# ZhengyiLuo/PULSE

Hardware: NVIDIA H100
Metric: env-steps/sec at 16384 humanoid envs, 1/2/4/8 H100; obs-kernel HBM GB/s (higher is better)
Workload: dtype bf16 GEMM operands, fp32 accumulate / master weights / observations

## Files before the change

pulse_b200/csrc/gemm_kernel.inc:

```
#if PULSE_GEMM_GROUPED
#define PULSE_GEMM_FIRST(member) grp.p[0].member
#define PULSE_GEMM_W wl
#define PULSE_GEMM_SELECT(w)                                                                                         \
  int pi = 0;                                                                                                        \
  while (pi + 1 < grp.count && (w) >= grp.p[pi].item_end) ++pi;                                                      \
  const GemmProblem& P = grp.p[pi];                                                                                  \
  const int wl = (w) - (pi == 0 ? 0 : grp.p[pi - 1].item_end);                                                       \
  const CUtensorMap& map_a = P.map_a;                                                                                \
  const CUtensorMap& map_b = P.map_b;                                                                                \
  const CUtensorMap& map_c = P.map_c;                                                                                \
  const int use_tma_red = P.use_tma_red;                                                                             \
  const pulse_gemm_epilogue_t& ep = P.ep;                                                                            \
  const int M = P.M, N = P.N, K = P.K, kb_per_split = P.kb_per_split;                                                \
  const int tiles_n = (N + BN - 1) / BN, tiles_m = (M + BM - 1) / BM;                                                \
  const int tiles = tiles_m * tiles_n;                                                                               \
  const int num_kb_total = (K + BK - 1) / BK;                                                                        \
  (void)map_a; (void)map_b; (void)map_c; (void)use_tma_red; (void)ep; (void)M; (void)N; (void)tiles_n; (void)kb_per_split; (void)num_kb_total;
#else
#define PULSE_GEMM_FIRST(member) member
#define PULSE_GEMM_W w
#define PULSE_GEMM_SELECT(w)
#endif

#if PULSE_GEMM_GROUPED
// ... 19 lines not shown
  const int work_stride = static_cast<int>(gridDim.x);
#if PULSE_GEMM_GROUPED
  const int total = grp.total_items;
#else
  const int tiles_n = (N + BN - 1) / BN, tiles_m = (M + BM - 1) / BM;
  const int tiles = tiles_m * tiles_n;
  const int total = tiles * splits;
  const int num_kb_total = (K + BK - 1) / BK;
#endif
  if (threadIdx.x == 0) PULSE_TRACE(0);

  if (threadIdx.x == 0) {
#pragma unroll
    for (int s = 0; s < kStages; ++s) {
      g_mbar_init(&sm.full[s], 1);
      g_mbar_init(&sm.empty[s], kConsumerWarps);
    }
    asm volatile("fence.mbarrier_init.release.cluster;\n" ::: "memory");
    asm volatile("prefetch.tensormap [%0];\n" ::"l"(&PULSE_GEMM_FIRST(map_a)) : "memory");
    asm volatile("prefetch.tensormap [%0];\n" ::"l"(&PULSE_GEMM_FIRST(map_b)) : "memory");
  }
  __syncthreads();
  if (threadIdx.x == 0) PULSE_TRACE(1);
  asm volatile("griddepcontrol.launch_dependents;\n" ::: "memory");

  if (warp < 4) {
    if (warp == 0 && lane == 0) {
      asm volatile("griddepcontrol.wait;\n" ::: "memory");
      PULSE_TRACE(2);
      int it = 0;
      for (int w = work0; w < total; w += work_stride) {
        PULSE_GEMM_SELECT(w)
        const int split = PULSE_GEMM_W / tiles, t = PULSE_GEMM_W - split * tiles;
        const int m0 = (t / tiles_n) * BM, n0 = (t % tiles_n) * BN;
        const int kb0 = split * kb_per_split;
        const int num_kb = min(kb_per_split, num_kb_total - kb0);
        for (int kb = 0; kb < num_kb; ++kb, ++it) {
          const int s = it % kStages;
          g_mbar_wait(&sm.empty[s], ((it / kStages) & 1) ^ 1);
          g_mbar_expect_tx(&sm.full[s], kStageBytesA + kStageBytesB);
          const int kk = (kb0 + kb) * BK;
// ... 1 lines not shown
            tma_load_2d(sm.a[s], &map_a, m0, kk, &sm.full[s]);
            tma_load_2d(sm.a[s] + 8192, &map_a, m0 + 64, kk, &sm.full[s]);
          } else {
            tma_load_2d(sm.a[s], &map_a, kk, m0, &sm.full[s]);
          }
          if (B_MN) {
            tma_load_2d(sm.b[s], &map_b, n0, kk, &sm.full[s]);
            tma_load_2d(sm.b[s] + 8192, &map_b, n0 + 64, kk, &sm.full[s]);
          } else {
            tma_load_2d(sm.b[s], &map_b, kk, n0, &sm.full[s]);
          }
        }
      }
    }
  } else {
    const int wg = (warp >> 2) - 1;
    const int ew = warp - 4;
    const int quarter = wg * 2 + (warp & 1);
    const int chalf = (warp >> 1) & 1;
    float* red_stage = sm.red[ew];
    float* acc_s = sm.acc[wg];
    asm volatile("griddepcontrol.wait;\n" ::: "memory");
    int it = 0, lw = 0;
    for (int w = work0; w < total; w += work_stride, ++lw) {
      PULSE_GEMM_SELECT(w)
      const int split = PULSE_GEMM_W / tiles, t = PULSE_GEMM_W - split * tiles;
      const int m0 = (t / tiles_n) * BM, n0 = (t % tiles_n) * BN;
      const int kb0 = split * kb_per_split;
      const int num_kb = min(kb_per_split, num_kb_total - kb0);
      const int row = m0 + quarter * 32 + lane;
      const bool row_ok = row < M;
      const bool gate_fast = (MODE == kModeGeneric || MODE == kModeDgrad) && ep.gate != nullptr && ep.gate_mask == nullptr && ep.gate_mode == PULSE_ACT_RELU && (ep.ldg & 7) == 0 && n0 + chalf * kCols + kCols <= N;
      unsigned gmask[kChunks] = {};
      const bool gate_bits = kDgrad && ep.gate_mask != nullptr;
      if (gate_bits && row_ok) {
#pragma unroll
        for (int cc = 0; cc < kChunks; ++cc) {
          const int col = n0 + (chalf * kChunks + cc) * 32;
          if (col < N) gmask[cc] = __ldg(ep.gate_mask + static_cast<long long>(col >> 5) * ep.ld_gmask + row);
        }
      }
      if (gate_fast && row_ok) {
        const uint4* g = reinterpret_cast<const uint4*>(reinterpret_cast<const __nv_bfloat16*>(ep.gate) + static_cast<long long>(row) * ep.ldg +
                                                        n0 + chalf * kCols);
        uint4 u[kChunks * 4];
#pragma unroll
        for (int i = 0; i < kChunks * 4; ++i) u[i] = __ldg(g + i);
#pragma unroll
        for (int i = 0; i < kChunks * 4; ++i) {
          const unsigned wds[4] = {u[i].x, u[i].y, u[i].z, u[i].w};
#pragma unroll
          for (int q = 0; q < 4; ++q) {
            const unsigned pos = (((wds[q] & 0x7fff7fffu) + 0x7fff7fffu) & ~wds[q]) & 0x80008000u;
            gmask[i >> 2] |= (pos >> 15) << ((i & 3) * 4 + q);
          }
        }
      }
      const bool gate_vec = kGateVec && ep.gate != nullptr && !gate_fast && !gate_bits && (ep.ldg & 7) == 0;
      uint4 gq[4] = {};
      auto gate_fetch = [&](int cc) {
        const int c0 = n0 + cc * 32;
        if (gate_vec && row_ok && c0 + 32 <= N) {
          const uint4* g = reinterpret_cast<const uint4*>(reinterpret_cast<const __nv_bfloat16*>(ep.gate) + static_cast<long long>(row) * ep.ldg + c0);
#pragma unroll
          for (int q = 0; q < 4; ++q) gq[q] = __ldg(g + q);
        }
      };
      gate_fetch(chalf * kChunks);
      float bias_l[kChunks] = {};
      const bool fwd_fast = MODE == kModeFwd && ep.out != nullptr && (ep.ldo & 7) == 0 && ep.out_f32 == nullptr && ep.out_t == nullptr &&
                            (ep.preact == nullptr || (ep.ldp & 7) == 0) && n0 + chalf * kCols + kCols <= N;
      float* bias_s = sm.bias[ew];
      if (fwd_fast && ep.bias != nullptr) {
        __syncwarp();
#pragma unroll
        for (int cc = 0; cc < kChunks; ++cc) bias_s[cc * 32 + lane] = __ldg(ep.bias + n0 + (chalf * kChunks + cc) * 32 + lane);
        __syncwarp();
      } else if (kFwd && ep.bias != nullptr) {
#pragma unroll
        for (int cc = 0; cc < kChunks; ++cc) {
          const int col = n0 + (chalf * kChunks + cc) * 32 + lane;
          if (col < N) bias_l[cc] = __ldg(ep.bias + col);
        }
      }

      float d[64];
#pragma unroll
      for (int i = 0; i < 64; ++i) d[i] = 0.0f;
      acc_fence(d);
      int prev_s = -1;
      for (int kb = 0; kb < num_kb; ++kb, ++it) {
        const int s = it % kStages;
        g_mbar_wait(&sm.full[s], (it / kStages) & 1);
        if (it == 0 && ew == 0 && lane == 0) PULSE_TRACE(3);
        wgmma_fence();
        const unsigned a_addr = s_u32(sm.a[s]) + static_cast<unsigned>(wg) * 8192u, b_addr = s_u32(sm.b[s]);
#pragma unroll
        for (int k = 0; k < BK / MMA_K; ++k) {
          const unsigned long long da = A_MN ? gmma_desc(a_addr + k * 2048, 8192) : gmma_desc(a_addr + k * 32, 16);
          const unsigned long long db = B_MN ? gmma_desc(b_addr + k * 2048, 8192) : gmma_desc(b_addr + k * 32, 16);
          wgmma_m64n128<A_MN ? 1 : 0, B_MN ? 1 : 0>(d, da, db, (kb | k) != 0 ? 1u : 0u);
        }
        wgmma_commit();
        wgmma_wait<1>();
        if (prev_s >= 0 && lane == 0) g_mbar_arrive(&sm.empty[prev_s]);
        prev_s = s;
      }
      wgmma_wait<0>();
      acc_fence(d);
      if (lane == 0) g_mbar_arrive(&sm.empty[prev_s]);
      if (ew == 0 && lane == 0 && lw < 3) PULSE_TRACE(4 + lw);

      wg_sync(wg);
      {
        const int r0 = (warp & 3) * 16 + (lane >> 2);
#pragma unroll
        for (int j = 0; j < BN / 8; ++j) {
          const int col = 8 * j + 2 * (lane & 3);
#pragma unroll
          for (int h = 0; h < 2; ++h) {
            const int r = r0 + 8 * h;
            const int rb = r & 31;
            float* blk = acc_s + ((r >> 5) * 4 + (col >> 5)) * 1024;
            const int unit = ((col & 31) >> 2) ^ (rb & 7);
            *reinterpret_cast<float2*>(blk + rb * 32 + unit * 4 + (col & 3)) = make_float2(d[4 * j + 2 * h], d[4 * j + 2 * h + 1]);
          }
        }
      }
      if (MODE == kModeWgrad && use_tma_red) asm volatile("fence.proxy.async.shared::cta;\n" ::: "memory");
      wg_sync(wg);
      if (ew == 0 && lane == 0 && lw < 3) PULSE_TRACE(16 + 2 * lw);

      float* outf = ep.out_f32 != nullptr ? ep.out_f32 + static_cast<long long>(ep.accumulate ? 0 : split) * ep.split_stride : nullptr;
      float sq = 0.0f;
#pragma unroll 1
      for (int c = chalf * kChunks; c < chalf * kChunks + kChunks; ++c) {
        const int col0 = n0 + c * 32;
        const bool full = col0 + 32 <= N;
        float* blk = acc_s + ((quarter & 1) * 4 + c) * 1024;
        if (MODE == kModeWgrad && use_tma_red) {
          if (lane == 0) {
            asm volatile("cp.reduce.async.bulk.tensor.2d.global.shared::cta.add.tile.bulk_group [%0, {%2, %3}], [%1];\n" ::"l"(&map_c),
                         "r"(s_u32(blk)), "r"(col0), "r"(m0 + quarter * 32)
                         : "memory");
            asm volatile("cp.async.bulk.commit_group;\n" ::: "memory");
          }
          continue;
        }
        float v[32];
        {
          const float4* b4 = reinterpret_cast<const float4*>(blk) + lane * 8;
#pragma unroll
          for (int u = 0; u < 8; ++u) {
            const float4 x = b4[u ^ (lane & 7)];
            v[4 * u] = x.x; v[4 * u + 1] = x.y; v[4 * u + 2] = x.z; v[4 * u + 3] = x.w;
          }
        }
        if (MODE != kModeWgrad && ep.alpha != 1.0f) {
#pragma unroll
          for (int i = 0; i < 32; ++i) v[i] *= ep.alpha;
        }
        if (fwd_fast) {
          if (ep.bias != nullptr) {
            const float4* b4 = reinterpret_cast<const float4*>(bias_s + (c % kChunks) * 32);
#pragma unroll
            for (int i = 0; i < 32; i += 4) {
              const float4 b = b4[i >> 2];
              v[i] += b.x; v[i + 1] += b.y; v[i + 2] += b.z; v[i + 3] += b.w;
            }
          }
          if (ep.relu_mask != nullptr) {
            unsigned word = 0u;
#pragma unroll
            for (int i = 0; i < 32; ++i) word |= (v[i] > 0.0f ? 1u : 0u) << i;
            if (row_ok) ep.relu_mask[static_cast<long long>(col0 >> 5) * ep.ld_rmask + row] = word;
          }
          uint4* st = reinterpret_cast<uint4*>(red_stage);
          const int sw = (lane >> 1) & 3;
#pragma unroll
          for (int q = 0; q < 4; ++q) {
            const int i = 8 * q;
            __nv_bfloat162 h0 = __floats2bfloat162_rn(v[i], v[i + 1]), h1 = __floats2bfloat162_rn(v[i + 2], v[i + 3]);
            __nv_bfloat162 h2 = __floats2bfloat162_rn(v[i + 4], v[i + 5]), h3 = __floats2bfloat162_rn(v[i + 6], v[i + 7]);
            uint4 u;
            u.x = *reinterpret_cast<unsigned*>(&h0);
            u.y = *reinterpret_cast<unsigned*>(&h1);
            u.z = *reinterpret_cast<unsigned*>(&h2);
            u.w = *reinterpret_cast<unsigned*>(&h3);
            st[lane * 4 + (q ^ sw)] = u;
          }
          __syncwarp();
          const long long coff = col0 + (lane & 3) * 8;
          const __nv_bfloat162 zero2 = __float2bfloat162_rn(0.0f);
#pragma unroll
          for (int it2 = 0; it2 < 4; ++it2) {
            const int rr = it2 * 8 + (lane >> 2);
            uint4 u = st[rr * 4 + ((lane & 3) ^ ((rr >> 1) & 3))];
            __nv_bfloat162* h = reinterpret_cast<__nv_bfloat162*>(&u);
            const long long grow = m0 + quarter * 32 + rr;
            if (grow < M) {
              if (ep.preact != nullptr) *reinterpret_cast<uint4*>(reinterpret_cast<__nv_bfloat16*>(ep.preact) + grow * ep.ldp + coff) = u;
              if (ep.act == PULSE_ACT_RELU) {
#pragma unroll
                for (int q = 0; q < 4; ++q) h[q] = __hmax2(h[q], zero2);
              } else if (ep.act == PULSE_ACT_SILU) {
#pragma unroll
                for (int q = 0; q < 4; ++q) h[q] = silu_bf16x2(h[q]);
              }
              *reinterpret_cast<uint4*>(reinterpret_cast<__nv_bfloat16*>(ep.out) + grow * ep.ldo + coff) = u;
            }
          }
          __syncwarp();
          continue;
        }
        if (kFwd && ep.bias != nullptr) {
          float bl = bias_l[0];
#pragma unroll
          for (int cc = 1; cc < kChunks; ++cc) bl = (c % kChunks) == cc ? bias_l[cc] : bl;
#pragma unroll
          for (int i = 0; i < 32; ++i) v[i] += __shfl_sync(0xffffffffu, bl, i);
        }
        if (kFwd && ep.preact != nullptr) {
          if (full && (ep.ldp & 7) == 0) {
            store_block_bf16(reinterpret_cast<uint4*>(red_stage), v,
                             reinterpret_cast<__nv_bfloat16*>(ep.preact) + static_cast<long long>(m0 + quarter * 32) * ep.ldp + col0, ep.ldp,
                             M - (m0 + quarter * 32), lane);
          } else if (row_ok) {
            __nv_bfloat16* p = reinterpret_cast<__nv_bfloat16*>(ep.preact) + static_cast<long long>(row) * ep.ldp + col0;
#pragma unroll
            for (int i = 0; i < 32; ++i)
              if (col0 + i < N) p[i] = __float2bfloat16(v[i]);
          }
        }
        if (kFwd && ep.relu_mask != nullptr && row_ok) {
          unsigned word = 0u;
#pragma unroll
          for (int i = 0; i < 32; ++i) word |= ((col0 + i < N && v[i] > 0.0f) ? 1u : 0u) << i;
          if (col0 < N) ep.relu_mask[static_cast<long long>(col0 >> 5) * ep.ld_rmask + row] = word;
        }
        if (kFwd && ep.act != PULSE_ACT_NONE) {
#pragma unroll
          for (int i = 0; i < 32; ++i) v[i] = act_apply(v[i], ep.act);
        }
        if (gate_bits) {
          unsigned mk = gmask[0];
#pragma unroll
          for (int cc = 1; cc < kChunks; ++cc) mk = (c % kChunks) == cc ? gmask[cc] : mk;
#pragma unroll
          for (int i = 0; i < 32; ++i) v[i] = ((mk >> i) & 1u) ? v[i] : 0.0f;
        } else if (gate_fast) {
          unsigned mk = gmask[0];
#pragma unroll
          for (int cc = 1; cc < kChunks; ++cc) mk = (c % kChunks) == cc ? gmask[cc] : mk;
#pragma unroll
          for (int i = 0; i < 32; ++i) v[i] = ((mk >> ((i >> 1) + 16 * (i & 1))) & 1u) ? v[i] : 0.0f;
        } else if (kDgrad && ep.gate != nullptr && row_ok) {
          const __nv_bfloat16* g = reinterpret_cast<const __nv_bfloat16*>(ep.gate) + static_cast<long long>(row) * ep.ldg + col0;
          if (full && (gate_vec || (ep.ldg & 7) == 0)) {
#pragma unroll
            for (int i = 0; i < 32; i += 8) {
              const uint4 u = gate_vec ? gq[i >> 3] : __ldg(reinterpret_cast<const uint4*>(g + i));
              const __nv_bfloat162* h = reinterpret_cast<const __nv_bfloat162*>(&u);
#pragma unroll
              for (int q = 0; q < 4; ++q) {
                const float2 f = __bfloat1622float2(h[q]);
                v[i + 2 * q] *= act_grad(f.x, ep.gate_mode);
                v[i + 2 * q + 1] *= act_grad(f.y, ep.gate_mode);
              }
            }
          } else {
#pragma unroll
            for (int i = 0; i < 32; ++i)
              if (col0 + i < N) v[i] *= act_grad(__bfloat162float(g[i]), ep.gate_mode);
          }
        }
        if (gate_vec && c != chalf * kChunks + kChunks - 1) gate_fetch(c + 1);
        if (kDgrad && ep.sumsq != nullptr && row_ok) {
#pragma unroll
          for (int i = 0; i < 32; ++i)
            if (full || col0 + i < N) sq = fmaf(v[i], v[i], sq);
        }
        if (kDgrad && ep.colsum != nullptr) {
          float wv[32];
#pragma unroll
          for (int i = 0; i < 32; ++i) wv[i] = row_ok ? v[i] : 0.0f;
#pragma unroll
          for (int half = 16; half >= 1; half >>= 1) {
            const bool upper = (lane & half) != 0;
#pragma unroll
            for (int i = 0; i < half; ++i) {
              const float mine = upper ? wv[i + half] : wv[i];
              const float send = upper ? wv[i] : wv[i + half];
              wv[i] = mine + __shfl_xor_sync(0xffffffffu, send, half);
            }
          }
          if (col0 + lane < N) atomicAdd(ep.colsum + col0 + lane, wv[0]);
        }
        if (kAccum && outf != nullptr && ep.accumulate) {
#pragma unroll
          for (int hr = 0; hr < 2; ++hr) {
            if ((lane >> 4) == hr) {
#pragma unroll
              for (int i = 0; i < 32; ++i) red_stage[(lane & 15) * 33 + i] = v[i];
            }
            __syncwarp();
            const int rbase = m0 + quarter * 32 + hr * 16;
            const int rows_here = min(16, M - rbase);
            if (col0 + lane < N) {
              float* p = outf + static_cast<long long>(rbase) * ep.ldf + col0 + lane;
              for (int rr = 0; rr < rows_here; ++rr) atomicAdd(p + static_cast<long long>(rr) * ep.ldf, red_stage[rr * 33 + lane]);
            }
            __syncwarp();
          }
        } else if (outf != nullptr && row_ok) {
          float* p = outf + static_cast<long long>(row) * ep.ldf + col0;
          if (full && (ep.ldf & 3) == 0 && (reinterpret_cast<uintptr_t>(outf) & 15u) == 0) {
#pragma unroll
            for (int i = 0; i < 32; i += 4) *reinterpret_cast<float4*>(p + i) = make_float4(v[i], v[i + 1], v[i + 2], v[i + 3]);
          } else {
#pragma unroll
            for (int i = 0; i < 32; ++i)
              if (col0 + i < N) p[i] = v[i];
          }
        }
        if (kBf16Out && ep.out != nullptr) {
          if (full && (ep.ldo & 7) == 0) {
            store_block_bf16(reinterpret_cast<uint4*>(red_stage), v,
                             reinterpret_cast<__nv_bfloat16*>(ep.out) + static_cast<long long>(m0 + quarter * 32) * ep.ldo + col0, ep.ldo,
                             M - (m0 + quarter * 32), lane);
          } else if (row_ok) {
            __nv_bfloat16* p = reinterpret_cast<__nv_bfloat16*>(ep.out) + static_cast<long long>(row) * ep.ldo + col0;
#pragma unroll
            for (int i = 0; i < 32; ++i)
              if (col0 + i < N) p[i] = __float2bfloat16(v[i]);
          }
        }
        if (kFwd && ep.out_t != nullptr && row_ok) {
#pragma unroll
          for (int i = 0; i < 32; ++i)
            if (col0 + i < N)
              reinterpret_cast<__nv_bfloat16*>(ep.out_t)[static_cast<long long>(col0 + i) * ep.ldot + row] = __float2bfloat16(v[i]);
        }
      }
      if (MODE == kModeWgrad && use_tma_red) {
        if (lane == 0) asm volatile("cp.async.bulk.wait_group.read 0;\n" ::: "memory");
        __syncwarp();
      }
      if (kDgrad && ep.sumsq != nullptr) {
#pragma unroll
        for (int o = 16; o > 0; o >>= 1) sq += __shfl_xor_sync(0xffffffffu, sq, o);
        if (lane == 0) atomicAdd(ep.sumsq, static_cast<double>(sq));
      }
      if (ew == 0 && lane == 0 && lw < 3) PULSE_TRACE(17 + 2 * lw);
    }
  }
  if (MODE == kModeWgrad && warp >= 4 && lane == 0) asm volatile("cp.async.bulk.wait_group 0;\n" ::: "memory");
  if (threadIdx.x == 0) PULSE_TRACE(10);
}


#undef PULSE_GEMM_FIRST
#undef PULSE_GEMM_W
#undef PULSE_GEMM_SELECT
```

pulse_b200/csrc/gemm_wgmma.cu:

```cuda
#include <cuda.h>
#include <stdlib.h>
#include <string.h>
#include <cuda_bf16.h>

#include "pulse_common.cuh"

namespace pulse {
namespace {

#ifndef PULSE_GEMM_VARIANT
#define PULSE_GEMM_VARIANT 0
#endif
constexpr int BM = 128, BN = 128, BK = 64, MMA_K = 16;
constexpr int kConsumerWarps = 8;
constexpr int kThreads = 128 + 32 * kConsumerWarps;
constexpr int kCols = 64;
constexpr int kChunks = kCols / 32;
constexpr int kStages = 4;
constexpr unsigned kStageBytesA = BM * BK * 2;
constexpr unsigned kStageBytesB = BN * BK * 2;

struct __align__(1024) GemmSmem {
  unsigned char a[kStages][kStageBytesA];
  unsigned char b[kStages][kStageBytesB];
  float acc[2][64 * BN];
  float red[kConsumerWarps][16 * 33];
  float bias[kConsumerWarps][kCols];
  unsigned long long full[kStages];
  unsigned long long empty[kStages];
};

__device__ __forceinline__ unsigned s_u32(const void* p) { return static_cast<unsigned>(__cvta_generic_to_shared(p)); }
__device__ __forceinline__ void g_mbar_init(unsigned long long* bar, unsigned count) {
  asm volatile("mbarrier.init.shared::cta.b64 [%0], %1;\n" ::"r"(s_u32(bar)), "r"(count));
}
__device__ __forceinline__ void g_mbar_expect_tx(unsigned long long* bar, unsigned bytes) {
  asm volatile("mbarrier.arrive.expect_tx.shared::cta.b64 _, [%0], %1;\n" ::"r"(s_u32(bar)), "r"(bytes) : "memory");
}
__device__ __forceinline__ void g_mbar_arrive(unsigned long long* bar) {
  asm volatile("mbarrier.arrive.shared::cta.b64 _, [%0];\n" ::"r"(s_u32(bar)) : "memory");
}
__device__ __forceinline__ bool g_mbar_try(unsigned long long* bar, unsigned parity) {
// ... 86 lines not shown
    u.z = *reinterpret_cast<unsigned*>(&h2);
    u.w = *reinterpret_cast<unsigned*>(&h3);
    st[lane * 4 + (q ^ sw)] = u;
  }
  __syncwarp();
  __nv_bfloat16* obase = base + (lane & 3) * 8;
#pragma unroll
  for (int it = 0; it < 4; ++it) {
    const int rr = it * 8 + (lane >> 2);
    const uint4 val = st[rr * 4 + ((lane & 3) ^ ((rr >> 1) & 3))];
    if (rr < rows_valid) *reinterpret_cast<uint4*>(obase + static_cast<long long>(rr) * ld) = val;
  }
  __syncwarp();
}

#if PULSE_GEMM_VARIANT == 3
__device__ long long g_gemm_trace[32];
#define PULSE_TRACE(slot)                                          \
  do {                                                             \
    if (blockIdx.x == 0) g_gemm_trace[slot] = clock64();           \
  } while (0)
#else
#define PULSE_TRACE(slot) \
  do {                    \
  } while (0)
#endif

__device__ __forceinline__ __nv_bfloat162 silu_bf16x2(__nv_bfloat162 z) {
  float2 f = __bfloat1622float2(z);
  f.x = __fdividef(f.x, 1.0f + __expf(-f.x));
// ... 52 lines not shown
bool make_map_c(CUtensorMap* map, const float* base, long long rows, long long cols, long long ld) {
  EncodeTiledFn fn = get_encode_fn();
  if (fn == nullptr) return false;
  cuuint64_t dims[2] = {static_cast<cuuint64_t>(cols), static_cast<cuuint64_t>(rows)};
  cuuint64_t strides[1] = {static_cast<cuuint64_t>(ld) * 4};
  cuuint32_t box[2] = {32, 32};
  cuuint32_t estr[2] = {1, 1};
  return fn(map, CU_TENSOR_MAP_DATA_TYPE_FLOAT32, 2, const_cast<float*>(base), dims, strides, box, estr, CU_TENSOR_MAP_INTERLEAVE_NONE,
            CU_TENSOR_MAP_SWIZZLE_128B, CU_TENSOR_MAP_L2_PROMOTION_NONE, CU_TENSOR_MAP_FLOAT_OOB_FILL_NONE) == CUDA_SUCCESS;
}
bool tma_reduce_ok(const pulse_gemm_epilogue_t& ep) {
  return ep.out_f32 != nullptr && ep.accumulate && (ep.ldf % 4) == 0 && (reinterpret_cast<uintptr_t>(ep.out_f32) % 16) == 0;
}

constexpr size_t kSmemBytes = sizeof(GemmSmem) + 1024;

int gemm_num_sms(bool honour_limit) {
  static int num_sms = 0, limited = 0;
  if (num_sms == 0) {
    int dev = 0;
    if (cudaGetDevice(&dev) != cudaSuccess || cudaDeviceGetAttribute(&num_sms, cudaDevAttrMultiProcessorCount, dev) != cudaSuccess) return 0;
    limited = num_sms;
    const char* e = getenv("PULSE_GEMM_SMS");
    if (e != nullptr && atoi(e) >= 1 && atoi(e) < num_sms) limited = atoi(e);
  }
  return honour_limit ? limited : num_sms;
}

template <bool A_MN, bool B_MN, int MODE>
int launch_gemm(const CUtensorMap& map_a, const CUtensorMap& map_b, const pulse_gemm_epilogue_t& ep, int m, int n, int k, int splits,
// ... 212 lines not shown
```

Before: 1.456 million.

## Ping-pong consumer warpgroups with 128-row tiles and register-direct epilogue

Each consumer warpgroup now handles whole alternating tiles and computes both 64-row halves (two accumulators) instead of splitting one tile across warpgroups. Named barriers order the two groups so one runs its MMAs while the other runs its epilogue. setmaxnreg moves registers from the producer to the consumers to fit the doubled accumulators. A new register-only epilogue for forward and dgrad writes bf16 outputs through quad shuffles without staging in shared memory, which also frees the red/bias shared buffers. The risks are register pressure or spills, and the change to the empty-barrier count and the barrier handshake must be correct.

```diff
diff --git a/pulse_b200/csrc/gemm_kernel.inc b/pulse_b200/csrc/gemm_kernel.inc
--- a/pulse_b200/csrc/gemm_kernel.inc
+++ b/pulse_b200/csrc/gemm_kernel.inc
@@ -57,7 +57,7 @@
 #pragma unroll
     for (int s = 0; s < kStages; ++s) {
       g_mbar_init(&sm.full[s], 1);
-      g_mbar_init(&sm.empty[s], kConsumerWarps);
+      g_mbar_init(&sm.empty[s], 4);
     }
     asm volatile("fence.mbarrier_init.release.cluster;\n" ::: "memory");
     asm volatile("prefetch.tensormap [%0];\n" ::"l"(&PULSE_GEMM_FIRST(map_a)) : "memory");
@@ -68,6 +68,7 @@
   asm volatile("griddepcontrol.launch_dependents;\n" ::: "memory");
 
   if (warp < 4) {
+    asm volatile("setmaxnreg.dec.sync.aligned.u32 %0;\n" ::"n"(kProducerRegs));
     if (warp == 0 && lane == 0) {
       asm volatile("griddepcontrol.wait;\n" ::: "memory");
       PULSE_TRACE(2);
@@ -99,11 +100,10 @@
       }
     }
   } else {
+    asm volatile("setmaxnreg.inc.sync.aligned.u32 %0;\n" ::"n"(kConsumerRegs));
     const int wg = (warp >> 2) - 1;
     const int ew = warp - 4;
-    const int quarter = wg * 2 + (warp & 1);
     const int chalf = (warp >> 1) & 1;
-    float* red_stage = sm.red[ew];
     float* acc_s = sm.acc[wg];
     asm volatile("griddepcontrol.wait;\n" ::: "memory");
     int it = 0, lw = 0;
@@ -113,330 +113,368 @@
       const int m0 = (t / tiles_n) * BM, n0 = (t % tiles_n) * BN;
       const int kb0 = split * kb_per_split;
       const int num_kb = min(kb_per_split, num_kb_total - kb0);
-      const int row = m0 + quarter * 32 + lane;
-      const bool row_ok = row < M;
-      const bool gate_fast = (MODE == kModeGeneric || MODE == kModeDgrad) && ep.gate != nullptr && ep.gate_mask == nullptr && ep.gate_mode == PULSE_ACT_RELU && (ep.ldg & 7) == 0 && n0 + chalf * kCols + kCols <= N;
-      unsigned gmask[kChunks] = {};
-      const bool gate_bits = kDgrad && ep.gate_mask != nullptr;
-      if (gate_bits && row_ok) {
-#pragma unroll
-        for (int cc = 0; cc < kChunks; ++cc) {
-          const int col = n0 + (chalf * kChunks + cc) * 32;
-          if (col < N) gmask[cc] = __ldg(ep.gate_mask + static_cast<long long>(col >> 5) * ep.ld_gmask + row);
-        }
-      }
-      if (gate_fast && row_ok) {
-        const uint4* g = reinterpret_cast<const uint4*>(reinterpret_cast<const __nv_bfloat16*>(ep.gate) + static_cast<long long>(row) * ep.ldg +
-                                                        n0 + chalf * kCols);
-        uint4 u[kChunks * 4];
-#pragma unroll
-        for (int i = 0; i < kChunks * 4; ++i) u[i] = __ldg(g + i);
-#pragma unroll
-        for (int i = 0; i < kChunks * 4; ++i) {
-          const unsigned wds[4] = {u[i].x, u[i].y, u[i].z, u[i].w};
-#pragma unroll
-          for (int q = 0; q < 4; ++q) {
-            const unsigned pos = (((wds[q] & 0x7fff7fffu) + 0x7fff7fffu) & ~wds[q]) & 0x80008000u;
-            gmask[i >> 2] |= (pos >> 15) << ((i & 3) * 4 + q);
-          }
-        }
-      }
-      const bool gate_vec = kGateVec && ep.gate != nullptr && !gate_fast && !gate_bits && (ep.ldg & 7) == 0;
-      uint4 gq[4] = {};
-      auto gate_fetch = [&](int cc) {
-        const int c0 = n0 + cc * 32;
-        if (gate_vec && row_ok && c0 + 32 <= N) {
-          const uint4* g = reinterpret_cast<const uint4*>(reinterpret_cast<const __nv_bfloat16*>(ep.gate) + static_cast<long long>(row) * ep.ldg + c0);
-#pragma unroll
-          for (int q = 0; q < 4; ++q) gq[q] = __ldg(g + q);
+      if ((lw & 1) != wg) {
+        it += num_kb;
+        continue;
+      }
+
+      const bool reg_fwd = MODE == kModeFwd && ep.out != nullptr && (ep.ldo & 7) == 0 && ep.out_f32 == nullptr && ep.out_t == nullptr &&
+                           (ep.preact == nullptr || (ep.ldp & 7) == 0) && n0 + BN <= N;
+      const bool reg_dgrad = MODE == kModeDgrad && ep.out != nullptr && (ep.ldo & 7) == 0 && ep.out_f32 == nullptr && ep.gate_mask != nullptr &&
+                             ep.gate == nullptr && ep.colsum == nullptr && ep.sumsq == nullptr && n0 + BN <= N;
+      const int row_r = m0 + 16 * (warp & 3) + (lane >> 2);
+      float2 bias2[BN / 8] = {};
+      unsigned gm[2][2][BN / 32] = {};
+      auto load_gate_words = [&](int half) {
+#pragma unroll
+        for (int hr = 0; hr < 2; ++hr) {
+          const int r = row_r + 64 * half + 8 * hr;
+#pragma unroll
+          for (int cc = 0; cc < BN / 32; ++cc)
+            if (r < M) gm[half][hr][cc] = __ldg(ep.gate_mask + static_cast<long long>((n0 >> 5) + cc) * ep.ld_gmask + r);
         }
       };
-      gate_fetch(chalf * kChunks);
-      float bias_l[kChunks] = {};
-      const bool fwd_fast = MODE == kModeFwd && ep.out != nullptr && (ep.ldo & 7) == 0 && ep.out_f32 == nullptr && ep.out_t == nullptr &&
-                            (ep.preact == nullptr || (ep.ldp & 7) == 0) && n0 + chalf * kCols + kCols <= N;
-      float* bias_s = sm.bias[ew];
-      if (fwd_fast && ep.bias != nullptr) {
-        __syncwarp();
-#pragma unroll
-        for (int cc = 0; cc < kChunks; ++cc) bias_s[cc * 32 + lane] = __ldg(ep.bias + n0 + (chalf * kChunks + cc) * 32 + lane);
-        __syncwarp();
-      } else if (kFwd && ep.bias != nullptr) {
-#pragma unroll
-        for (int cc = 0; cc < kChunks; ++cc) {
-          const int col = n0 + (chalf * kChunks + cc) * 32 + lane;
-          if (col < N) bias_l[cc] = __ldg(ep.bias + col);
-        }
-      }
-
-      float d[64];
-#pragma unroll
-      for (int i = 0; i < 64; ++i) d[i] = 0.0f;
-      acc_fence(d);
+      if (reg_fwd && ep.bias != nullptr) {
+#pragma unroll
+        for (int j = 0; j < BN / 8; ++j) bias2[j] = make_float2(__ldg(ep.bias + n0 + 8 * j + 2 * (lane & 3)), __ldg(ep.bias + n0 + 8 * j + 2 * (lane & 3) + 1));
+      }
+      if (reg_dgrad) load_gate_words(0);
+
+      float d0[64], d1[64];
+#pragma unroll
+      for (int i = 0; i < 64; ++i) d0[i] = d1[i] = 0.0f;
+      acc_fence(d0);
+      acc_fence(d1);
+      if (lw > 0) asm volatile("bar.sync %0, 256;\n" ::"r"(3 + wg) : "memory");
+      if ((ew & 3) == 0 && lane == 0 && lw < 3) PULSE_TRACE(11 + lw);
       int prev_s = -1;
       for (int kb = 0; kb < num_kb; ++kb, ++it) {
         const int s = it % kStages;
         g_mbar_wait(&sm.full[s], (it / kStages) & 1);
         if (it == 0 && ew == 0 && lane == 0) PULSE_TRACE(3);
         wgmma_fence();
-        const unsigned a_addr = s_u32(sm.a[s]) + static_cast<unsigned>(wg) * 8192u, b_addr = s_u32(sm.b[s]);
+        const unsigned a_addr = s_u32(sm.a[s]), b_addr = s_u32(sm.b[s]);
 #pragma unroll
         for (int k = 0; k < BK / MMA_K; ++k) {
-          const unsigned long long da = A_MN ? gmma_desc(a_addr + k * 2048, 8192) : gmma_desc(a_addr + k * 32, 16);
+          const unsigned long long da0 = A_MN ? gmma_desc(a_addr + k * 2048, 8192) : gmma_desc(a_addr + k * 32, 16);
+          const unsigned long long da1 = A_MN ? gmma_desc(a_addr + 8192 + k * 2048, 8192) : gmma_desc(a_addr + 8192 + k * 32, 16);
           const unsigned long long db = B_MN ? gmma_desc(b_addr + k * 2048, 8192) : gmma_desc(b_addr + k * 32, 16);
-          wgmma_m64n128<A_MN ? 1 : 0, B_MN ? 1 : 0>(d, da, db, (kb | k) != 0 ? 1u : 0u);
+          wgmma_m64n128<A_MN ? 1 : 0, B_MN ? 1 : 0>(d0, da0, db, (kb | k) != 0 ? 1u : 0u);
+          wgmma_m64n128<A_MN ? 1 : 0, B_MN ? 1 : 0>(d1, da1, db, (kb | k) != 0 ? 1u : 0u);
         }
         wgmma_commit();
         wgmma_wait<1>();
         if (prev_s >= 0 && lane == 0) g_mbar_arrive(&sm.empty[prev_s]);
         prev_s = s;
       }
+      if (w + work_stride < total) asm volatile("bar.arrive %0, 256;\n" ::"r"(3 + (wg ^ 1)) : "memory");
       wgmma_wait<0>();
-      acc_fence(d);
+      acc_fence(d0);
+      acc_fence(d1);
       if (lane == 0) g_mbar_arrive(&sm.empty[prev_s]);
-      if (ew == 0 && lane == 0 && lw < 3) PULSE_TRACE(4 + lw);
-
-      wg_sync(wg);
-      {
-        const int r0 = (warp & 3) * 16 + (lane >> 2);
-#pragma unroll
-        for (int j = 0; j < BN / 8; ++j) {
-          const int col = 8 * j + 2 * (lane & 3);
-#pragma unroll
-          for (int h = 0; h < 2; ++h) {
-            const int r = r0 + 8 * h;
-            const int rb = r & 31;
-            float* blk = acc_s + ((r >> 5) * 4 + (col >> 5)) * 1024;
-            const int unit = ((col & 31) >> 2) ^ (rb & 7);
-            *reinterpret_cast<float2*>(blk + rb * 32 + unit * 4 + (col & 3)) = make_float2(d[4 * j + 2 * h], d[4 * j + 2 * h + 1]);
-          }
-        }
-      }
-      if (MODE == kModeWgrad && use_tma_red) asm volatile("fence.proxy.async.shared::cta;\n" ::: "memory");
-      wg_sync(wg);
-      if (ew == 0 && lane == 0 && lw < 3) PULSE_TRACE(16 + 2 * lw);
-
-      float* outf = ep.out_f32 != nullptr ? ep.out_f32 + static_cast<long long>(ep.accumulate ? 0 : split) * ep.split_stride : nullptr;
-      float sq = 0.0f;
+      if ((ew & 3) == 0 && lane == 0 && lw < 3) PULSE_TRACE(4 + lw);
+
+      if (MODE == kModeFwd || MODE == kModeDgrad) {
+        if (reg_fwd || reg_dgrad) {
+          if (reg_dgrad) load_gate_words(1);
+          epilogue_regs<MODE == kModeFwd>(d0, bias2, gm[0], ep, row_r, n0, M, lane);
+          epilogue_regs<MODE == kModeFwd>(d1, bias2, gm[1], ep, row_r + 64, n0, M, lane);
+          if ((ew & 3) == 0 && lane == 0 && lw < 3) PULSE_TRACE(17 + 2 * lw);
+          continue;
+        }
+      }
+
 #pragma unroll 1
-      for (int c = chalf * kChunks; c < chalf * kChunks + kChunks; ++c) {
-        const int col0 = n0 + c * 32;
-        const bool full = col0 + 32 <= N;
-        float* blk = acc_s + ((quarter & 1) * 4 + c) * 1024;
+      for (int h = 0; h < 2; ++h) {
+        const int quarter = h * 2 + (warp & 1);
+        const int row = m0 + quarter * 32 + lane;
+        const bool row_ok = row < M;
+        const bool gate_fast = (MODE == kModeGeneric || MODE == kModeDgrad) && ep.gate != nullptr && ep.gate_mask == nullptr && ep.gate_mode == PULSE_ACT_RELU && (ep.ldg & 7) == 0 && n0 + chalf * kCols + kCols <= N;
+        unsigned gmask[kChunks] = {};
+        const bool gate_bits = kDgrad && ep.gate_mask != nullptr;
+        if (gate_bits && row_ok) {
+#pragma unroll
+          for (int cc = 0; cc < kChunks; ++cc) {
+            const int col = n0 + (chalf * kChunks + cc) * 32;
+            if (col < N) gmask[cc] = __ldg(ep.gate_mask + static_cast<long long>(col >> 5) * ep.ld_gmask + row);
+          }
+        }
+        if (gate_fast && row_ok) {
+          const uint4* g = reinterpret_cast<const uint4*>(reinterpret_cast<const __nv_bfloat16*>(ep.gate) + static_cast<long long>(row) * ep.ldg +
+                                                          n0 + chalf * kCols);
+          uint4 u[kChunks * 4];
+#pragma unroll
+          for (int i = 0; i < kChunks * 4; ++i) u[i] = __ldg(g + i);
+#pragma unroll
+          for (int i = 0; i < kChunks * 4; ++i) {
+            const unsigned wds[4] = {u[i].x, u[i].y, u[i].z, u[i].w};
+#pragma unroll
+            for (int q = 0; q < 4; ++q) {
+              const unsigned pos = (((wds[q] & 0x7fff7fffu) + 0x7fff7fffu) & ~wds[q]) & 0x80008000u;
+              gmask[i >> 2] |= (pos >> 15) << ((i & 3) * 4 + q);
+            }
+          }
+        }
+        const bool gate_vec = kGateVec && ep.gate != nullptr && !gate_fast && !gate_bits && (ep.ldg & 7) == 0;
+        uint4 gq[4] = {};
+        auto gate_fetch = [&](int cc) {
+          const int c0 = n0 + cc * 32;
+          if (gate_vec && row_ok && c0 + 32 <= N) {
+            const uint4* g = reinterpret_cast<const uint4*>(reinterpret_cast<const __nv_bfloat16*>(ep.gate) + static_cast<long long>(row) * ep.ldg + c0);
+#pragma unroll
+            for (int q = 0; q < 4; ++q) gq[q] = __ldg(g + q);
+          }
+        };
+        gate_fetch(chalf * kChunks);
+        float bias_l[kChunks] = {};
+        const bool fwd_fast = MODE == kModeFwd && ep.out != nullptr && (ep.ldo & 7) == 0 && ep.out_f32 == nullptr && ep.out_t == nullptr &&
+                              (ep.preact == nullptr || (ep.ldp & 7) == 0) && n0 + chalf * kCols + kCols <= N;
+        if (kFwd && ep.bias != nullptr) {
+#pragma unroll
+          for (int cc = 0; cc < kChunks; ++cc) {
+            const int col = n0 + (chalf * kChunks + cc) * 32 + lane;
+            if (col < N) bias_l[cc] = __ldg(ep.bias + col);
+          }
+        }
+
+        wg_sync(wg);
+        {
+          const int r0 = (warp & 3) * 16 + (lane >> 2);
+#pragma unroll
+          for (int j = 0; j < BN / 8; ++j) {
+            const int col = 8 * j + 2 * (lane & 3);
+#pragma unroll
+            for (int hr = 0; hr < 2; ++hr) {
+              const int r = r0 + 8 * hr;
+              const int rb = r & 31;
+              float* blk = acc_s + ((r >> 5) * 4 + (col >> 5)) * 1024;
+              const int unit = ((col & 31) >> 2) ^ (rb & 7);
+              *reinterpret_cast<float2*>(blk + rb * 32 + unit * 4 + (col & 3)) = make_float2(d0[4 * j + 2 * hr], d0[4 * j + 2 * hr + 1]);
+            }
+          }
+        }
+        if (MODE == kModeWgrad && use_tma_red) asm volatile("fence.proxy.async.shared::cta;\n" ::: "memory");
+        wg_sync(wg);
+        if ((ew & 3) == 0 && lane == 0 && lw < 3 && h == 0) PULSE_TRACE(16 + 2 * lw);
+
+        float* outf = ep.out_f32 != nullptr ? ep.out_f32 + static_cast<long long>(ep.accumulate ? 0 : split) * ep.split_stride : nullptr;
+        float sq = 0.0f;
+#pragma unroll 1
+        for (int c = chalf * kChunks; c < chalf * kChunks + kChunks; ++c) {
+          const int col0 = n0 + c * 32;
+          const bool full = col0 + 32 <= N;
+          float* blk = acc_s + ((quarter & 1) * 4 + c) * 1024;
+          if (MODE == kModeWgrad && use_tma_red) {
+            if (lane == 0) {
+              asm volatile("cp.reduce.async.bulk.tensor.2d.global.shared::cta.add.tile.bulk_group [%0, {%2, %3}], [%1];\n" ::"l"(&map_c),
+                           "r"(s_u32(blk)), "r"(col0), "r"(m0 + quarter * 32)
+                           : "memory");
+              asm volatile("cp.async.bulk.commit_group;\n" ::: "memory");
+            }
+            continue;
+          }
+          float v[32];
+          {
+            const float4* b4 = reinterpret_cast<const float4*>(blk) + lane * 8;
+#pragma unroll
+            for (int u = 0; u < 8; ++u) {
+              const float4 x = b4[u ^ (lane & 7)];
+              v[4 * u] = x.x; v[4 * u + 1] = x.y; v[4 * u + 2] = x.z; v[4 * u + 3] = x.w;
+            }
+          }
+          float* red_stage = blk;
+          __syncwarp();
+          if (MODE != kModeWgrad && ep.alpha != 1.0f) {
+#pragma unroll
+            for (int i = 0; i < 32; ++i) v[i] *= ep.alpha;
+          }
+          if (kFwd && ep.bias != nullptr) {
+            float bl = bias_l[0];
+#pragma unroll
+            for (int cc = 1; cc < kChunks; ++cc) bl = (c % kChunks) == cc ? bias_l[cc] : bl;
+#pragma unroll
+            for (int i = 0; i < 32; ++i) v[i] += __shfl_sync(0xffffffffu, bl, i);
+          }
+          if (fwd_fast) {
+            if (ep.relu_mask != nullptr) {
+              unsigned word = 0u;
+#pragma unroll
+              for (int i = 0; i < 32; ++i) word |= (v[i] > 0.0f ? 1u : 0u) << i;
+              if (row_ok) ep.relu_mask[static_cast<long long>(col0 >> 5) * ep.ld_rmask + row] = word;
+            }
+            uint4* st = reinterpret_cast<uint4*>(red_stage);
+            const int sw = (lane >> 1) & 3;
+#pragma unroll
+            for (int q = 0; q < 4; ++q) {
+              const int i = 8 * q;
+              __nv_bfloat162 h0 = __floats2bfloat162_rn(v[i], v[i + 1]), h1 = __floats2bfloat162_rn(v[i + 2], v[i + 3]);
+              __nv_bfloat162 h2 = __floats2bfloat162_rn(v[i + 4], v[i + 5]), h3 = __floats2bfloat162_rn(v[i + 6], v[i + 7]);
+              uint4 u;
+              u.x = *reinterpret_cast<unsigned*>(&h0);
+              u.y = *reinterpret_cast<unsigned*>(&h1);
+              u.z = *reinterpret_cast<unsigned*>(&h2);
+              u.w = *reinterpret_cast<unsigned*>(&h3);
+              st[lane * 4 + (q ^ sw)] = u;
+            }
+            __syncwarp();
+            const long long coff = col0 + (lane & 3) * 8;
+            const __nv_bfloat162 zero2 = __float2bfloat162_rn(0.0f);
+#pragma unroll
+            for (int it2 = 0; it2 < 4; ++it2) {
+              const int rr = it2 * 8 + (lane >> 2);
+              uint4 u = st[rr * 4 + ((lane & 3) ^ ((rr >> 1) & 3))];
+              __nv_bfloat162* h = reinterpret_cast<__nv_bfloat162*>(&u);
+              const long long grow = m0 + quarter * 32 + rr;
+              if (grow < M) {
+                if (ep.preact != nullptr) *reinterpret_cast<uint4*>(reinterpret_cast<__nv_bfloat16*>(ep.preact) + grow * ep.ldp + coff) = u;
+                if (ep.act == PULSE_ACT_RELU) {
+#pragma unroll
+                  for (int q = 0; q < 4; ++q) h[q] = __hmax2(h[q], zero2);
+                } else if (ep.act == PULSE_ACT_SILU) {
+#pragma unroll
+                  for (int q = 0; q < 4; ++q) h[q] = silu_bf16x2(h[q]);
+                }
+                *reinterpret_cast<uint4*>(reinterpret_cast<__nv_bfloat16*>(ep.out) + grow * ep.ldo + coff) = u;
+              }
+            }
+            __syncwarp();
+            continue;
+          }
+          if (kFwd && ep.preact != nullptr) {
+            if (full && (ep.ldp & 7) == 0) {
+              store_block_bf16(reinterpret_cast<uint4*>(red_stage), v,
+                               reinterpret_cast<__nv_bfloat16*>(ep.preact) + static_cast<long long>(m0 + quarter * 32) * ep.ldp + col0, ep.ldp,
+                               M - (m0 + quarter * 32), lane);
+            } else if (row_ok) {
+              __nv_bfloat16* p = reinterpret_cast<__nv_bfloat16*>(ep.preact) + static_cast<long long>(row) * ep.ldp + col0;
+#pragma unroll
+              for (int i = 0; i < 32; ++i)
+                if (col0 + i < N) p[i] = __float2bfloat16(v[i]);
+            }
+          }
+          if (kFwd && ep.relu_mask != nullptr && row_ok) {
+            unsigned word = 0u;
+#pragma unroll
+            for (int i = 0; i < 32; ++i) word |= ((col0 + i < N && v[i] > 0.0f) ? 1u : 0u) << i;
+            if (col0 < N) ep.relu_mask[static_cast<long long>(col0 >> 5) * ep.ld_rmask + row] = word;
+          }
+          if (kFwd && ep.act != PULSE_ACT_NONE) {
+#pragma unroll
+            for (int i = 0; i < 32; ++i) v[i] = act_apply(v[i], ep.act);
+          }
+          if (gate_bits) {
+            unsigned mk = gmask[0];
+#pragma unroll
+            for (int cc = 1; cc < kChunks; ++cc) mk = (c % kChunks) == cc ? gmask[cc] : mk;
+#pragma unroll
+            for (int i = 0; i < 32; ++i) v[i] = ((mk >> i) & 1u) ? v[i] : 0.0f;
+          } else if (gate_fast) {
+            unsigned mk = gmask[0];
+#pragma unroll
+            for (int cc = 1; cc < kChunks; ++cc) mk = (c % kChunks) == cc ? gmask[cc] : mk;
+#pragma unroll
+            for (int i = 0; i < 32; ++i) v[i] = ((mk >> ((i >> 1) + 16 * (i & 1))) & 1u) ? v[i] : 0.0f;
+          } else if (kDgrad && ep.gate != nullptr && row_ok) {
+            const __nv_bfloat16* g = reinterpret_cast<const __nv_bfloat16*>(ep.gate) + static_cast<long long>(row) * ep.ldg + col0;
+            if (full && (gate_vec || (ep.ldg & 7) == 0)) {
+#pragma unroll
+              for (int i = 0; i < 32; i += 8) {
+                const uint4 u = gate_vec ? gq[i >> 3] : __ldg(reinterpret_cast<const uint4*>(g + i));
+                const __nv_bfloat162* h = reinterpret_cast<const __nv_bfloat162*>(&u);
+#pragma unroll
+                for (int q = 0; q < 4; ++q) {
+                  const float2 f = __bfloat1622float2(h[q]);
+                  v[i + 2 * q] *= act_grad(f.x, ep.gate_mode);
+                  v[i + 2 * q + 1] *= act_grad(f.y, ep.gate_mode);
+                }
+              }
+            } else {
+#pragma unroll
+              for (int i = 0; i < 32; ++i)
+                if (col0 + i < N) v[i] *= act_grad(__bfloat162float(g[i]), ep.gate_mode);
+            }
+          }
+          if (gate_vec && c != chalf * kChunks + kChunks - 1) gate_fetch(c + 1);
+          if (kDgrad && ep.sumsq != nullptr && row_ok) {
+#pragma unroll
+            for (int i = 0; i < 32; ++i)
+              if (full || col0 + i < N) sq = fmaf(v[i], v[i], sq);
+          }
+          if (kDgrad && ep.colsum != nullptr) {
+            float wv[32];
+#pragma unroll
+            for (int i = 0; i < 32; ++i) wv[i] = row_ok ? v[i] : 0.0f;
+#pragma unroll
+            for (int half = 16; half >= 1; half >>= 1) {
+              const bool upper = (lane & half) != 0;
+#pragma unroll
+              for (int i = 0; i < half; ++i) {
+                const float mine = upper ? wv[i + half] : wv[i];
+                const float send = upper ? wv[i] : wv[i + half];
+                wv[i] = mine + __shfl_xor_sync(0xffffffffu, send, half);
+              }
+            }
+            if (col0 + lane < N) atomicAdd(ep.colsum + col0 + lane, wv[0]);
+          }
+          if (kAccum && outf != nullptr && ep.accumulate) {
+#pragma unroll
+            for (int hr = 0; hr < 2; ++hr) {
+              if ((lane >> 4) == hr) {
+#pragma unroll
+                for (int i = 0; i < 32; ++i) red_stage[(lane & 15) * 33 + i] = v[i];
+              }
+              __syncwarp();
+              const int rbase = m0 + quarter * 32 + hr * 16;
+              const int rows_here = min(16, M - rbase);
+              if (col0 + lane < N) {
+                float* p = outf + static_cast<long long>(rbase) * ep.ldf + col0 + lane;
+                for (int rr = 0; rr < rows_here; ++rr) atomicAdd(p + static_cast<long long>(rr) * ep.ldf, red_stage[rr * 33 + lane]);
+              }
+              __syncwarp();
+            }
+          } else if (outf != nullptr && row_ok) {
+            float* p = outf + static_cast<long long>(row) * ep.ldf + col0;
+            if (full && (ep.ldf & 3) == 0 && (reinterpret_cast<uintptr_t>(outf) & 15u) == 0) {
+#pragma unroll
+              for (int i = 0; i < 32; i += 4) *reinterpret_cast<float4*>(p + i) = make_float4(v[i], v[i + 1], v[i + 2], v[i + 3]);
+            } else {
+#pragma unroll
+              for (int i = 0; i < 32; ++i)
+                if (col0 + i < N) p[i] = v[i];
+            }
+          }
+          if (kBf16Out && ep.out != nullptr) {
+            if (full && (ep.ldo & 7) == 0) {
+              store_block_bf16(reinterpret_cast<uint4*>(red_stage), v,
+                               reinterpret_cast<__nv_bfloat16*>(ep.out) + static_cast<long long>(m0 + quarter * 32) * ep.ldo + col0, ep.ldo,
+                               M - (m0 + quarter * 32), lane);
+            } else if (row_ok) {
+              __nv_bfloat16* p = reinterpret_cast<__nv_bfloat16*>(ep.out) + static_cast<long long>(row) * ep.ldo + col0;
+#pragma unroll
+              for (int i = 0; i < 32; ++i)
+                if (col0 + i < N) p[i] = __float2bfloat16(v[i]);
+            }
+          }
+          if (kFwd && ep.out_t != nullptr && row_ok) {
+#pragma unroll
+            for (int i = 0; i < 32; ++i)
+              if (col0 + i < N)
+                reinterpret_cast<__nv_bfloat16*>(ep.out_t)[static_cast<long long>(col0 + i) * ep.ldot + row] = __float2bfloat16(v[i]);
+          }
+        }
         if (MODE == kModeWgrad && use_tma_red) {
-          if (lane == 0) {
-            asm volatile("cp.reduce.async.bulk.tensor.2d.global.shared::cta.add.tile.bulk_group [%0, {%2, %3}], [%1];\n" ::"l"(&map_c),
-                         "r"(s_u32(blk)), "r"(col0), "r"(m0 + quarter * 32)
-                         : "memory");
-            asm volatile("cp.async.bulk.commit_group;\n" ::: "memory");
-          }
-          continue;
-        }
-        float v[32];
-        {
-          const float4* b4 = reinterpret_cast<const float4*>(blk) + lane * 8;
-#pragma unroll
-          for (int u = 0; u < 8; ++u) {
-            const float4 x = b4[u ^ (lane & 7)];
-            v[4 * u] = x.x; v[4 * u + 1] = x.y; v[4 * u + 2] = x.z; v[4 * u + 3] = x.w;
-          }
-        }
-        if (MODE != kModeWgrad && ep.alpha != 1.0f) {
-#pragma unroll
-          for (int i = 0; i < 32; ++i) v[i] *= ep.alpha;
-        }
-        if (fwd_fast) {
-          if (ep.bias != nullptr) {
-            const float4* b4 = reinterpret_cast<const float4*>(bias_s + (c % kChunks) * 32);
-#pragma unroll
-            for (int i = 0; i < 32; i += 4) {
-              const float4 b = b4[i >> 2];
-              v[i] += b.x; v[i + 1] += b.y; v[i + 2] += b.z; v[i + 3] += b.w;
-            }
-          }
-          if (ep.relu_mask != nullptr) {
-            unsigned word = 0u;
-#pragma unroll
-            for (int i = 0; i < 32; ++i) word |= (v[i] > 0.0f ? 1u : 0u) << i;
-            if (row_ok) ep.relu_mask[static_cast<long long>(col0 >> 5) * ep.ld_rmask + row] = word;
-          }
-          uint4* st = reinterpret_cast<uint4*>(red_stage);
-          const int sw = (lane >> 1) & 3;
-#pragma unroll
-          for (int q = 0; q < 4; ++q) {
-            const int i = 8 * q;
-            __nv_bfloat162 h0 = __floats2bfloat162_rn(v[i], v[i + 1]), h1 = __floats2bfloat162_rn(v[i + 2], v[i + 3]);
-            __nv_bfloat162 h2 = __floats2bfloat162_rn(v[i + 4], v[i + 5]), h3 = __floats2bfloat162_rn(v[i + 6], v[i + 7]);
-            uint4 u;
-            u.x = *reinterpret_cast<unsigned*>(&h0);
-            u.y = *reinterpret_cast<unsigned*>(&h1);
-            u.z = *reinterpret_cast<unsigned*>(&h2);
-            u.w = *reinterpret_cast<unsigned*>(&h3);
-            st[lane * 4 + (q ^ sw)] = u;
-          }
+          if (lane == 0) asm volatile("cp.async.bulk.wait_group.read 0;\n" ::: "memory");
           __syncwarp();
-          const long long coff = col0 + (lane & 3) * 8;
-          const __nv_bfloat162 zero2 = __float2bfloat162_rn(0.0f);
-#pragma unroll
-          for (int it2 = 0; it2 < 4; ++it2) {
-            const int rr = it2 * 8 + (lane >> 2);
-            uint4 u = st[rr * 4 + ((lane & 3) ^ ((rr >> 1) & 3))];
-            __nv_bfloat162* h = reinterpret_cast<__nv_bfloat162*>(&u);
-            const long long grow = m0 + quarter * 32 + rr;
-            if (grow < M) {
-              if (ep.preact != nullptr) *reinterpret_cast<uint4*>(reinterpret_cast<__nv_bfloat16*>(ep.preact) + grow * ep.ldp + coff) = u;
-              if (ep.act == PULSE_ACT_RELU) {
-#pragma unroll
-                for (int q = 0; q < 4; ++q) h[q] = __hmax2(h[q], zero2);
-              } else if (ep.act == PULSE_ACT_SILU) {
-#pragma unroll
-                for (int q = 0; q < 4; ++q) h[q] = silu_bf16x2(h[q]);
-              }
-              *reinterpret_cast<uint4*>(reinterpret_cast<__nv_bfloat16*>(ep.out) + grow * ep.ldo + coff) = u;
-            }
-          }
-          __syncwarp();
-          continue;
-        }
-        if (kFwd && ep.bias != nullptr) {
-          float bl = bias_l[0];
-#pragma unroll
-          for (int cc = 1; cc < kChunks; ++cc) bl = (c % kChunks) == cc ? bias_l[cc] : bl;
-#pragma unroll
-          for (int i = 0; i < 32; ++i) v[i] += __shfl_sync(0xffffffffu, bl, i);
-        }
-        if (kFwd && ep.preact != nullptr) {
-          if (full && (ep.ldp & 7) == 0) {
-            store_block_bf16(reinterpret_cast<uint4*>(red_stage), v,
-                             reinterpret_cast<__nv_bfloat16*>(ep.preact) + static_cast<long long>(m0 + quarter * 32) * ep.ldp + col0, ep.ldp,
-                             M - (m0 + quarter * 32), lane);
-          } else if (row_ok) {
-            __nv_bfloat16* p = reinterpret_cast<__nv_bfloat16*>(ep.preact) + static_cast<long long>(row) * ep.ldp + col0;
-#pragma unroll
-            for (int i = 0; i < 32; ++i)
-              if (col0 + i < N) p[i] = __float2bfloat16(v[i]);
-          }
-        }
-        if (kFwd && ep.relu_mask != nullptr && row_ok) {
-          unsigned word = 0u;
-#pragma unroll
-          for (int i = 0; i < 32; ++i) word |= ((col0 + i < N && v[i] > 0.0f) ? 1u : 0u) << i;
-          if (col0 < N) ep.relu_mask[static_cast<long long>(col0 >> 5) * ep.ld_rmask + row] = word;
-        }
-        if (kFwd && ep.act != PULSE_ACT_NONE) {
-#pragma unroll
-          for (int i = 0; i < 32; ++i) v[i] = act_apply(v[i], ep.act);
-        }
-        if (gate_bits) {
-          unsigned mk = gmask[0];
-#pragma unroll
-          for (int cc = 1; cc < kChunks; ++cc) mk = (c % kChunks) == cc ? gmask[cc] : mk;
-#pragma unroll
-          for (int i = 0; i < 32; ++i) v[i] = ((mk >> i) & 1u) ? v[i] : 0.0f;
-        } else if (gate_fast) {
-          unsigned mk = gmask[0];
-#pragma unroll
-          for (int cc = 1; cc < kChunks; ++cc) mk = (c % kChunks) == cc ? gmask[cc] : mk;
-#pragma unroll
-          for (int i = 0; i < 32; ++i) v[i] = ((mk >> ((i >> 1) + 16 * (i & 1))) & 1u) ? v[i] : 0.0f;
-        } else if (kDgrad && ep.gate != nullptr && row_ok) {
-          const __nv_bfloat16* g = reinterpret_cast<const __nv_bfloat16*>(ep.gate) + static_cast<long long>(row) * ep.ldg + col0;
-          if (full && (gate_vec || (ep.ldg & 7) == 0)) {
-#pragma unroll
-            for (int i = 0; i < 32; i += 8) {
-              const uint4 u = gate_vec ? gq[i >> 3] : __ldg(reinterpret_cast<const uint4*>(g + i));
-              const __nv_bfloat162* h = reinterpret_cast<const __nv_bfloat162*>(&u);
-#pragma unroll
-              for (int q = 0; q < 4; ++q) {
-                const float2 f = __bfloat1622float2(h[q]);
-                v[i + 2 * q] *= act_grad(f.x, ep.gate_mode);
-                v[i + 2 * q + 1] *= act_grad(f.y, ep.gate_mode);
-              }
-            }
-          } else {
-#pragma unroll
-            for (int i = 0; i < 32; ++i)
-              if (col0 + i < N) v[i] *= act_grad(__bfloat162float(g[i]), ep.gate_mode);
-          }
-        }
-        if (gate_vec && c != chalf * kChunks + kChunks - 1) gate_fetch(c + 1);
-        if (kDgrad && ep.sumsq != nullptr && row_ok) {
-#pragma unroll
-          for (int i = 0; i < 32; ++i)
-            if (full || col0 + i < N) sq = fmaf(v[i], v[i], sq);
-        }
-        if (kDgrad && ep.colsum != nullptr) {
-          float wv[32];
-#pragma unroll
-          for (int i = 0; i < 32; ++i) wv[i] = row_ok ? v[i] : 0.0f;
-#pragma unroll
-          for (int half = 16; half >= 1; half >>= 1) {
-            const bool upper = (lane & half) != 0;
-#pragma unroll
-            for (int i = 0; i < half; ++i) {
-              const float mine = upper ? wv[i + half] : wv[i];
-              const float send = upper ? wv[i] : wv[i + half];
-              wv[i] = mine + __shfl_xor_sync(0xffffffffu, send, half);
-            }
-          }
-          if (col0 + lane < N) atomicAdd(ep.colsum + col0 + lane, wv[0]);
-        }
-        if (kAccum && outf != nullptr && ep.accumulate) {
-#pragma unroll
-          for (int hr = 0; hr < 2; ++hr) {
-            if ((lane >> 4) == hr) {
-#pragma unroll
-              for (int i = 0; i < 32; ++i) red_stage[(lane & 15) * 33 + i] = v[i];
-            }
-            __syncwarp();
-            const int rbase = m0 + quarter * 32 + hr * 16;
-            const int rows_here = min(16, M - rbase);
-            if (col0 + lane < N) {
-              float* p = outf + static_cast<long long>(rbase) * ep.ldf + col0 + lane;
-              for (int rr = 0; rr < rows_here; ++rr) atomicAdd(p + static_cast<long long>(rr) * ep.ldf, red_stage[rr * 33 + lane]);
-            }
-            __syncwarp();
-          }
-        } else if (outf != nullptr && row_ok) {
-          float* p = outf + static_cast<long long>(row) * ep.ldf + col0;
-          if (full && (ep.ldf & 3) == 0 && (reinterpret_cast<uintptr_t>(outf) & 15u) == 0) {
-#pragma unroll
-            for (int i = 0; i < 32; i += 4) *reinterpret_cast<float4*>(p + i) = make_float4(v[i], v[i + 1], v[i + 2], v[i + 3]);
-          } else {
-#pragma unroll
-            for (int i = 0; i < 32; ++i)
-              if (col0 + i < N) p[i] = v[i];
-          }
-        }
-        if (kBf16Out && ep.out != nullptr) {
-          if (full && (ep.ldo & 7) == 0) {
-            store_block_bf16(reinterpret_cast<uint4*>(red_stage), v,
-                             reinterpret_cast<__nv_bfloat16*>(ep.out) + static_cast<long long>(m0 + quarter * 32) * ep.ldo + col0, ep.ldo,
-                             M - (m0 + quarter * 32), lane);
-          } else if (row_ok) {
-            __nv_bfloat16* p = reinterpret_cast<__nv_bfloat16*>(ep.out) + static_cast<long long>(row) * ep.ldo + col0;
-#pragma unroll
-            for (int i = 0; i < 32; ++i)
-              if (col0 + i < N) p[i] = __float2bfloat16(v[i]);
-          }
-        }
-        if (kFwd && ep.out_t != nullptr && row_ok) {
-#pragma unroll
-          for (int i = 0; i < 32; ++i)
-            if (col0 + i < N)
-              reinterpret_cast<__nv_bfloat16*>(ep.out_t)[static_cast<long long>(col0 + i) * ep.ldot + row] = __float2bfloat16(v[i]);
-        }
-      }
-      if (MODE == kModeWgrad && use_tma_red) {
-        if (lane == 0) asm volatile("cp.async.bulk.wait_group.read 0;\n" ::: "memory");
-        __syncwarp();
-      }
-      if (kDgrad && ep.sumsq != nullptr) {
-#pragma unroll
-        for (int o = 16; o > 0; o >>= 1) sq += __shfl_xor_sync(0xffffffffu, sq, o);
-        if (lane == 0) atomicAdd(ep.sumsq, static_cast<double>(sq));
-      }
-      if (ew == 0 && lane == 0 && lw < 3) PULSE_TRACE(17 + 2 * lw);
+        }
+        if (kDgrad && ep.sumsq != nullptr) {
+#pragma unroll
+          for (int o = 16; o > 0; o >>= 1) sq += __shfl_xor_sync(0xffffffffu, sq, o);
+          if (lane == 0) atomicAdd(ep.sumsq, static_cast<double>(sq));
+        }
+#pragma unroll
+        for (int i = 0; i < 64; ++i) d0[i] = d1[i];
+      }
+      if ((ew & 3) == 0 && lane == 0 && lw < 3) PULSE_TRACE(17 + 2 * lw);
     }
   }
   if (MODE == kModeWgrad && warp >= 4 && lane == 0) asm volatile("cp.async.bulk.wait_group 0;\n" ::: "memory");
diff --git a/pulse_b200/csrc/gemm_wgmma.cu b/pulse_b200/csrc/gemm_wgmma.cu
--- a/pulse_b200/csrc/gemm_wgmma.cu
+++ b/pulse_b200/csrc/gemm_wgmma.cu
@@ -17,6 +17,7 @@
 constexpr int kCols = 64;
 constexpr int kChunks = kCols / 32;
 constexpr int kStages = 4;
+constexpr int kProducerRegs = 40, kConsumerRegs = 232;
 constexpr unsigned kStageBytesA = BM * BK * 2;
 constexpr unsigned kStageBytesB = BN * BK * 2;
 
@@ -24,8 +25,6 @@
   unsigned char a[kStages][kStageBytesA];
   unsigned char b[kStages][kStageBytesB];
   float acc[2][64 * BN];
-  float red[kConsumerWarps][16 * 33];
-  float bias[kConsumerWarps][kCols];
   unsigned long long full[kStages];
   unsigned long long empty[kStages];
 };
@@ -142,6 +141,80 @@
   __syncwarp();
 }
 
+__device__ __forceinline__ __nv_bfloat162 silu_bf16x2(__nv_bfloat162 z);
+
+__device__ __forceinline__ void quad_transpose(unsigned (&w)[4], int q) {
+#pragma unroll
+  for (int k = 0; k < 4; k += 2) {
+    const unsigned r = __shfl_xor_sync(0xffffffffu, (q & 1) ? w[k] : w[k + 1], 1);
+    if (q & 1) w[k] = r; else w[k + 1] = r;
+  }
+#pragma unroll
+  for (int k = 0; k < 2; ++k) {
+    const unsigned r = __shfl_xor_sync(0xffffffffu, (q & 2) ? w[k] : w[k + 2], 2);
+    if (q & 2) w[k] = r; else w[k + 2] = r;
+  }
+}
+
+template <bool FWD>
+__device__ __forceinline__ void epilogue_regs(const float (&d)[64], const float2 (&bias2)[BN / 8], const unsigned (&gmask)[2][BN / 32],
+                                              const pulse_gemm_epilogue_t& ep, int row0, int n0, int M, int lane) {
+  const int q = lane & 3;
+  const __nv_bfloat162 zero2 = __float2bfloat162_rn(0.0f);
+#pragma unroll
+  for (int hr = 0; hr < 2; ++hr) {
+    const long long row = row0 + 8 * hr;
+    const bool row_ok = row < M;
+#pragma unroll
+    for (int cc = 0; cc < BN / 32; ++cc) {
+      unsigned w[4], bits = 0u;
+#pragma unroll
+      for (int jj = 0; jj < 4; ++jj) {
+        const int j = 4 * cc + jj, b = 8 * jj + 2 * q;
+        float x0 = d[4 * j + 2 * hr], x1 = d[4 * j + 2 * hr + 1];
+        if (ep.alpha != 1.0f) {
+          x0 *= ep.alpha;
+          x1 *= ep.alpha;
+        }
+        if (FWD) {
+          if (ep.bias != nullptr) {
+            x0 += bias2[j].x;
+            x1 += bias2[j].y;
+          }
+          bits |= (x0 > 0.0f ? 1u : 0u) << b | (x1 > 0.0f ? 1u : 0u) << (b + 1);
+        } else {
+          x0 = ((gmask[hr][cc] >> b) & 1u) ? x0 : 0.0f;
+          x1 = ((gmask[hr][cc] >> (b + 1)) & 1u) ? x1 : 0.0f;
+        }
+        __nv_bfloat162 h = __floats2bfloat162_rn(x0, x1);
+        w[jj] = *reinterpret_cast<unsigned*>(&h);
+      }
+      if (FWD && ep.relu_mask != nullptr) {
+        bits |= __shfl_xor_sync(0xffffffffu, bits, 1);
+        bits |= __shfl_xor_sync(0xffffffffu, bits, 2);
+        if (q == cc && row_ok) ep.relu_mask[static_cast<long long>((n0 >> 5) + cc) * ep.ld_rmask + row] = bits;
+      }
+      quad_transpose(w, q);
+      uint4 u = make_uint4(w[0], w[1], w[2], w[3]);
+      const long long col = n0 + 32 * cc + 8 * q;
+      if (row_ok) {
+        if (FWD) {
+          if (ep.preact != nullptr) *reinterpret_cast<uint4*>(reinterpret_cast<__nv_bfloat16*>(ep.preact) + row * ep.ldp + col) = u;
+          __nv_bfloat162* h = reinterpret_cast<__nv_bfloat162*>(&u);
+          if (ep.act == PULSE_ACT_RELU) {
+#pragma unroll
+            for (int i = 0; i < 4; ++i) h[i] = __hmax2(h[i], zero2);
+          } else if (ep.act == PULSE_ACT_SILU) {
+#pragma unroll
+            for (int i = 0; i < 4; ++i) h[i] = silu_bf16x2(h[i]);
+          }
+        }
+        *reinterpret_cast<uint4*>(reinterpret_cast<__nv_bfloat16*>(ep.out) + row * ep.ldo + col) = u;
+      }
+    }
+  }
+}
+
 #if PULSE_GEMM_VARIANT == 3
 __device__ long long g_gemm_trace[32];
 #define PULSE_TRACE(slot)                                          \
@@ -224,6 +297,7 @@
 }
 
 constexpr size_t kSmemBytes = sizeof(GemmSmem) + 1024;
+static_assert(kSmemBytes <= 227 * 1024, "GEMM shared memory exceeds the 227 KB a block may use");
 
 int gemm_num_sms(bool honour_limit) {
   static int num_sms = 0, limited = 0;
```

Measured after the change: 1.508 million, median of 6. 1.04x the previous value.
